# GuildOfWeavers/distaff

Measured on AMD Instinct MI355X. Metric: trace_cells_per_sec, higher is better.
Workload: dtype u128 (prime field 2^128-45*2^40+1, 4x u32 limbs)

## Files before the change

### distaff_amd/csrc/air_kernel.h

```cpp
#pragma once
#include "ctx.h"
#include <type_traits>

#ifndef AIR_THREADS
#define AIR_THREADS 128
#endif
#ifdef AIR_CONVOY
#define AIR_SYNC() __builtin_amdgcn_s_barrier()
#else
#define AIR_SYNC()
#endif
#ifndef AIR_WAVES_PER_SIMD
#define AIR_WAVES_PER_SIMD 2
#endif
constexpr int air_waves_per_simd(int sd, int slcap, int sect) {
    (void)sd; (void)slcap; (void)sect;
#ifdef AIR_WAVES_FORCE
    return AIR_WAVES_FORCE;
#else
    return AIR_WAVES_PER_SIMD;
#endif
}

struct AirConsts { fe sponge_mds[16], sponge_inv_mds[16], hasher_mds[36], hasher_inv_mds[36]; };

struct AirArgs {
    const fe* lde;
    fe* out;
    const fe* coef;
    const fe* tc;
    const fe* periodic;
    const AirConsts* consts;
    fe* partial;
    fe* ev[10];
    const fe* tw_lo; const fe* tw_hi; uint32_t lo_bits;
    unsigned long long* bad_step;
    size_t n, col_stride;
    uint32_t log_n, log_N, log_b, W, ctx_depth, loop_depth, stack_depth;
    uint32_t cl, ll, sl;
    uint32_t coset_step;
    uint32_t q0;
    uint32_t num_inputs, num_outputs;
    fe inputs[8], outputs[8], program_hash[2], op_count;
};



__device__ __forceinline__ fe dpow(const AirArgs& a, uint64_t e) {
    uint32_t l = (uint32_t)e & ((1u << a.lo_bits) - 1u), h = (uint32_t)(e >> a.lo_bits);
    fe v = a.tw_lo[l];
    return h ? fe_mul(v, a.tw_hi[h]) : v;
}

__device__ __forceinline__ fe bnot(const fe& v) { return fe_sub(fe_one(), v); }
__device__ __forceinline__ fe is_bin(const fe& v) { return fe_sub(fe_sqr(v), v); }

template <int Wd>
__device__ __forceinline__ void matmul(fe* s, const fe* m) {
    fe r[Wd];
#pragma unroll
    for (int i = 0; i < Wd; i++) {
        fe_acc A; fe_acc_zero(A);
#pragma unroll
        for (int j = 0; j < Wd; j++) fe_acc_mac(A, m[i * Wd + j], s[j]);
        r[i] = fe_acc_reduce(A);
    }
#pragma unroll
    for (int i = 0; i < Wd; i++) s[i] = r[i];
}

template <int I, int N, class F>
__device__ __forceinline__ void static_for_air(F&& f) {
    if constexpr (I < N) { f(std::integral_constant<int, I>{}); static_for_air<I + 1, N>(f); }
}

struct StackRows { fe o[12], nw[8], hd0; int sl; };
#define ST_AUX0 8
#define ST_AUX1 9

template <int OP, int I> constexpr bool st_has() {
    constexpr bool slot = I < 8, aux0 = I == ST_AUX0, aux1 = I == ST_AUX1;
    switch (OP) {
        case 0x00: case 0x01: case 0x05: case 0x06: case 0x07: return slot || aux0;
        case 0x02: case 0x0E: return slot || aux0;
        case 0x03: case 0x04: case 0x08: case 0x09: case 0x0C: case 0x0D: return slot;
        case 0x0A: case 0x0B: return slot || aux0 || aux1;
        case 0x10: return I >= 1 && slot;
        case 0x11: return I >= 2 && slot;
        case 0x12: case 0x13: case 0x14: case 0x15: return slot;
        case 0x18: return slot && I != 1;
        case 0x19: case 0x1A: case 0x1B: case 0x1C: case 0x1D: return slot;
        default: return false;
    }
}

template <int OP, int I>
__device__ __forceinline__ fe st_term(const StackRows& s) {
    const fe* o = s.o; const fe* nw = s.nw;
    constexpr int i = I < 8 ? I : 0;
    auto L = [&](int num) {
        if (i + num < 8) return fe_sub(o[i + num < 8 ? i + num : 0], nw[i]);
        return i + num < s.sl ? fe_sub(o[i + num < 12 ? i + num : 0], nw[i]) : nw[i];
    };
    auto R = [&](int num) { return fe_sub(o[i - num < 0 ? 0 : i - num], nw[i]); };
    auto C = [&]() { return fe_sub(o[i], nw[i]); };
    auto sel = [&](const fe& c, const fe& x, const fe& y) { return fe_add(y, fe_mul(c, fe_sub(x, y))); };
    if constexpr (OP == 0x00) { if constexpr (I == ST_AUX0) return bnot(o[0]); else return L(1); }
    else if constexpr (OP == 0x01) { if constexpr (I == ST_AUX0) return fe_sub(o[0], o[1]); else return L(2); }
    else if constexpr (OP == 0x02) {
        const fe diff = fe_sub(o[1], o[2]);
        if constexpr (I == ST_AUX0) return fe_mul(nw[0], diff);
        else if constexpr (I == 0) return fe_sub(nw[0], bnot(fe_mul(diff, o[0])));
        else return L(2);
    }
    else if constexpr (OP == 0x03) return L(1);
    else if constexpr (OP == 0x04) return L(4);
    else if constexpr (OP == 0x05) {
        if constexpr (I == ST_AUX0) return is_bin(o[2]);
        else if constexpr (I == 0) return fe_sub(nw[0], sel(o[2], o[0], o[1]));
        else return L(2);
    }
    else if constexpr (OP == 0x06) {
        if constexpr (I == ST_AUX0) return is_bin(o[4]);
        else if constexpr (I == 0) return fe_sub(nw[0], sel(o[4], o[0], o[2]));
// ... 151 lines not shown
        }
        if constexpr ((GROUPS & (AG_RESCR | AG_KEEP)) != 0) {
            const fe keep = fe_sub(o[I < 8 ? I : 0], nw[I < 8 ? I : 0]);
            if constexpr ((GROUPS & AG_RESCR) != 0) { if constexpr (I < 6) fe_acc_mac(outer, h.rescr, h.resc[I < 6 ? I : 0]); else fe_acc_mac(outer, h.rescr, keep); }
            if constexpr ((GROUPS & AG_KEEP) != 0) fe_acc_mac(outer, h.keep, keep);
        }
    }
}

template <int I, uint32_t GROUPS> constexpr bool st_touches() {
    if (I >= 8) return (GROUPS & AG_LOW0) != 0;
    return (GROUPS & (AG_LOW0 | AG_LOW1 | AG_HIGH)) != 0;
}

template <int I, uint32_t GROUPS, int SDK, bool DEEP>
__device__ __forceinline__ fe st_output(const StackRows& s, const fe* lo2, const fe& lo0h, const fe* mid, const fe* top, const StackHigh& h) {
    fe_acc outer; fe_acc_zero(outer);
    static_for_air<0, 2>([&](auto c_) {
        constexpr int c = decltype(c_)::value;
        if constexpr (((GROUPS >> (4 * c)) & 0xFu) != 0) {
            fe_acc middle; fe_acc_zero(middle);
            static_for_air<0, 4>([&](auto b_) {
                constexpr int b = decltype(b_)::value;
                constexpr int base = 4 * b + 16 * c;
                if constexpr ((GROUPS & AG_LOW(c, b)) != 0) {
                    static constexpr StMerge M = st_merge<base, I, SDK, DEEP>();
                    if constexpr (M.n > 0) {
                        fe_acc inner; fe_acc_zero(inner);
                        static_for_air<0, M.n>([&](auto e_) {
                            constexpr int e = decltype(e_)::value;
                            fe cf = (base == 0 && M.lead[e] == 0) ? lo0h : lo2[M.lead[e]];
                            static_for_air<0, 4>([&](auto a_) {
                                constexpr int a = decltype(a_)::value;
                                if constexpr (a != M.lead[e] && M.sgn[e][a] != 0) {
                                    const fe other = (base == 0 && a == 0) ? lo0h : lo2[a];
                                    cf = M.sgn[e][a] > 0 ? fe_add(cf, other) : fe_sub(cf, other);
                                }
                            });
                            constexpr int ii = I < 8 ? I : 0;
                            fe term;
                            if constexpr (M.kind[e] == 1) term = fe_sub(s.o[M.j[e]], s.nw[ii]);
                            else if constexpr (M.kind[e] == 2) term = fe_sub(s.nw[ii], s.o[M.j[e]]);
                            else if constexpr (M.kind[e] == 3) term = s.nw[ii];
                            else if constexpr (M.kind[e] == 4) term = fe_neg(s.nw[ii]);
                            else term = st_term<base + M.lead[e], I>(s);
                            fe_acc_mac(inner, cf, term);
                        });
                        fe_acc_mac(middle, mid[b], fe_acc_reduce(inner));
                    }
                }
            });
            fe_acc_mac(outer, top[c], fe_acc_reduce(middle));
        }
    });
    if constexpr ((GROUPS & AG_HIGH) != 0) st_high_degree<I, GROUPS>(outer, s, h);
    return fe_acc_reduce(outer);
}

template <uint32_t ACC_MASK>
struct Acc {
    fe_acc res_acc;
    fe_acc adj_acc[6];
    fe res, adj[6];
    bool nonzero;
    const fe* tc; uint32_t nc;
    __device__ __forceinline__ void emit(uint32_t cidx, int slot, const fe& d) {
        nonzero |= !fe_is_zero(d);
        fe_acc_mac(res_acc, d, tc[cidx]);
        if ((ACC_MASK >> slot) & 1u) fe_acc_mac(adj_acc[slot], d, tc[nc + cidx]);
        else adj[slot] = fe_add(adj[slot], fe_mul(d, tc[nc + cidx]));
    }
};

template <int CL, int LL, int SD, int SLCAP, int SECT, uint32_t GROUPS, int FLAGS>
__global__ void __launch_bounds__(AIR_THREADS, air_waves_per_simd(SD, SLCAP, SECT)) air_kernel(AirArgs a) {
    constexpr bool FIRST = (FLAGS & AF_FIRST) != 0, LAST = (FLAGS & AF_LAST) != 0, EV_IN = (FLAGS & AF_EV_IN) != 0, EV_OUT = (FLAGS & AF_EV_OUT) != 0;
    constexpr int SL = SD ? (SD > 8 ? SD : 8) : SLCAP;
    constexpr bool DEEP = SD == 0 && SLCAP == 12;
    const int cl = (int)a.cl, ll = (int)a.ll;
    const int sl = SD ? SL : (int)a.sl;
    const int sd = SD ? SD : (int)a.stack_depth;
    const fe* c_sponge_mds = a.consts->sponge_mds; const fe* c_sponge_inv_mds = a.consts->sponge_inv_mds;
    const fe* c_hasher_mds = a.consts->hasher_mds; const fe* c_hasher_inv_mds = a.consts->hasher_inv_mds;
    const size_t k = (size_t)blockIdx.x * AIR_THREADS + threadIdx.x;
    if (k >= a.n) return;
    const uint32_t ql = blockIdx.y;
    const uint32_t qg = a.q0 + ql;
    const uint32_t jl = ql * a.coset_step;
    const size_t kn = (k + 1 == a.n) ? 0 : k + 1;
    const fe* cur_p = a.lde + (size_t)jl * a.n + k;
    const fe* nxt_p = a.lde + (size_t)jl * a.n + kn;
    const size_t cs = a.col_stride;
#define CUR(c) cur_p[(size_t)(c) * cs]
#define NXT(c) nxt_p[(size_t)(c) * cs]

    const uint64_t nmask = ((uint64_t)1 << a.log_N) - 1;
    const uint64_t gi = ((uint64_t)k << a.log_b) + (uint64_t)qg * a.coset_step;
    const uint32_t step = (uint32_t)(((uint64_t)k << 3) + qg);
    const uint64_t n64 = a.n;

    const fe c_opc = CUR(0), n_opc = NXT(0);
    fe c_sp[4], n_sp[4], cf[3], ld[5], hd[2], n_cf[3];
#pragma unroll
    for (int i = 0; i < 4; i++) { c_sp[i] = CUR(1 + i); n_sp[i] = NXT(1 + i); }
#pragma unroll
    for (int i = 0; i < 3; i++) { cf[i] = CUR(5 + i); n_cf[i] = NXT(5 + i); }
#pragma unroll
    for (int i = 0; i < 5; i++) ld[i] = CUR(8 + i);
#pragma unroll
    for (int i = 0; i < 2; i++) hd[i] = CUR(13 + i);
    fe c_ctx[CL], n_ctx[CL], c_lp[LL], n_lp[LL], o[SL], nw[SL];
    {
        uint32_t col = 15;
#pragma unroll
        for (int i = 0; i < CL; i++) { bool on = (uint32_t)i < a.ctx_depth; c_ctx[i] = on ? CUR(col + i) : fe_zero(); n_ctx[i] = on ? NXT(col + i) : fe_zero(); }
        col += a.ctx_depth;
#pragma unroll
        for (int i = 0; i < LL; i++) { bool on = (uint32_t)i < a.loop_depth; c_lp[i] = on ? CUR(col + i) : fe_zero(); n_lp[i] = on ? NXT(col + i) : fe_zero(); }
        col += a.loop_depth;
#pragma unroll
        for (int i = 0; i < SL; i++) { bool on = i < sd; o[i] = on ? CUR(col + i) : fe_zero(); nw[i] = on ? NXT(col + i) : fe_zero(); }
    }

    if constexpr ((SECT & 1) != 0) {
        const fe xp = dpow(a, (gi * (6 * n64 + 2)) & nmask);
        const fe one = fe_one();
#pragma unroll 1
        for (int pass = 0; pass < 2; pass++) {
            const fe* cc = a.coef + pass * 94;
            fe_acc R, A; fe_acc_zero(R); fe_acc_zero(A);
            auto term = [&](const fe& v, uint32_t idx) { fe_acc_mac(R, v, cc[idx]); fe_acc_mac(A, v, cc[idx + 1]); };
            term(pass ? fe_sub(c_opc, a.op_count) : c_opc, 0);
            if (pass == 0) { for (int i = 0; i < 4; i++) term(c_sp[i], 2 + 2 * i); }
            else { for (int i = 0; i < 2; i++) term(fe_sub(c_sp[i], a.program_hash[i]), 2 + 2 * i); }
            for (int i = 0; i < 3; i++) term(pass ? fe_sub(cf[i], one) : cf[i], 10 + 2 * i);
            for (int i = 0; i < 5; i++) term(pass ? fe_sub(ld[i], one) : ld[i], 16 + 2 * i);
            for (int i = 0; i < 2; i++) term(pass ? fe_sub(hd[i], one) : hd[i], 26 + 2 * i);
            for (int i = 0; i < CL; i++) if (i < cl) term(c_ctx[i], 30 + 2 * i);
            for (int i = 0; i < LL; i++) if (i < ll) term(c_lp[i], 62 + 2 * i);
            const uint32_t nio = pass ? a.num_outputs : a.num_inputs;
#pragma unroll
            for (int i = 0; i < 8; i++) if ((uint32_t)i < nio) term(fe_sub(o[i], pass ? a.outputs[i] : a.inputs[i]), 78 + 2 * i);
            const fe adj = fe_acc_reduce(A);
            fe_acc_mac(R, adj, xp);
            a.out[((size_t)pass * gridDim.y + ql) * a.n + k] = fe_acc_reduce(R);
        }
    }

    AIR_SYNC();
    fe cff[8], hdf[4], begin_flag, noop_flag, n_void, assert_flag;
    fe lo2[4], mid[4], top[2];
    {
        fe n0 = bnot(cf[0]), n1 = bnot(cf[1]), n2 = bnot(cf[2]);
        fe t0 = fe_mul(n0, n1), t1 = fe_mul(cf[0], n1), t2 = fe_mul(n0, cf[1]), t3 = fe_mul(cf[0], cf[1]);
        cff[0] = fe_mul(t0, n2); cff[1] = fe_mul(t1, n2); cff[2] = fe_mul(t2, n2); cff[3] = fe_mul(t3, n2);
        cff[4] = fe_mul(t0, cf[2]); cff[5] = fe_mul(t1, cf[2]); cff[6] = fe_mul(t2, cf[2]); cff[7] = fe_mul(t3, cf[2]);
        n_void = fe_mul(fe_mul(n_cf[0], n_cf[1]), n_cf[2]);
        fe l0 = bnot(ld[0]), l1 = bnot(ld[1]), l2 = bnot(ld[2]), l3 = bnot(ld[3]);
        lo2[0] = fe_mul(l0, l1); lo2[1] = fe_mul(ld[0], l1);
        lo2[2] = fe_mul(l0, cf[1]);
        lo2[3] = fe_mul(ld[0], ld[1]);
        mid[0] = fe_mul(l2, l3); mid[1] = fe_mul(ld[2], l3); mid[2] = fe_mul(l2, ld[3]); mid[3] = fe_mul(ld[2], ld[3]);
        top[0] = bnot(ld[4]); top[1] = ld[4];
        fe h0 = bnot(hd[0]), h1 = bnot(hd[1]);
        hdf[0] = fe_mul(h0, h1); hdf[1] = fe_mul(hd[0], h1); hdf[2] = fe_mul(h0, hd[1]); hdf[3] = fe_mul(hd[0], hd[1]);
    }
    auto LDF = [&](int idx) { return fe_mul(fe_mul(lo2[idx & 3], mid[(idx >> 2) & 3]), top[idx >> 4]); };
// ... 319 lines not shown
#pragma unroll
            for (int i = 0; i < 6; i++) agg(i, f, fe_sub(ns[i], os[i]));
            copy_from(6, f);
        }
        }

        const uint32_t sbase = 20 + cl + ll;
        if constexpr ((SECT & 40) != 0) { acc.emit(sbase, 4, aux0); acc.emit(sbase + 1, 4, aux1); }
#pragma unroll
        for (int i = 0; i < SLR; i++) if (i < sd) acc.emit(sbase + 2 + i, 4, ev[i]);
    }
    if constexpr (DEEP && (GROUPS & AG_DEEP) != 0) {
        {
            const uint32_t sbase = 20 + cl + ll;
            const fe lo_all = fe_add(fe_add(lo2[0], lo2[1]), fe_add(lo2[2], lo2[3]));
            fe fl1, fl2, fl4, fr1, fr2, fr4, fcp;
            { fe_acc A; fe_acc_zero(A); fe_acc_mac(A, mid[0], lo2[3]); fe_acc_mac(A, mid[2], lo_all); fl1 = fe_add(fe_mul(top[0], fe_acc_reduce(A)), assert_flag); }
            { fe_acc A; fe_acc_zero(A); fe_acc_mac(A, mid[0], fe_add(lo2[1], lo2[2])); fe_acc_mac(A, mid[1], fe_add(lo2[1], lo2[3])); fl2 = fe_mul(top[0], fe_acc_reduce(A)); }
            fl4 = fe_mul(top[0], fe_mul(mid[1], fe_add(lo2[0], lo2[2])));
            fr1 = fe_add(fe_mul(top[1], fe_mul(mid[0], fe_add(lo2[0], lo2[2]))), hdf[0]);
            { fe_acc A; fe_acc_zero(A); fe_acc_mac(A, mid[0], fe_add(lo2[1], lo2[3])); fe_acc_mac(A, mid[1], lo2[1]); fr2 = fe_mul(top[1], fe_acc_reduce(A)); }
            fr4 = fe_mul(top[1], fe_mul(mid[1], lo2[0]));
            {
                fe_acc A; fe_acc_zero(A); fe_acc_mac(A, mid[2], lo_all); fe_acc_mac(A, mid[3], fe_add(lo2[0], lo2[1]));
                fe_acc B; fe_acc_zero(B); fe_acc_mac(B, top[1], fe_acc_reduce(A)); fe_acc_mac(B, top[0], fe_mul(mid[3], fe_add(fe_add(lo2[0], lo2[1]), lo2[2])));
                fcp = fe_add(fe_add(fe_acc_reduce(B), fe_add(hdf[1], hdf[2])), fe_add(begin_flag, noop_flag));
            }
            const uint32_t scol = 15 + a.ctx_depth + a.loop_depth;
#pragma unroll 1
            for (int i = 8; i < sd; i++) {
                const fe ni = NXT(scol + i);
                auto item = [&](int j) { return CUR(scol + j); };
                auto left = [&](int num) { return i + num < sl ? fe_sub(item(i + num), ni) : ni; };
                fe_acc A; fe_acc_zero(A);
                fe_acc_mac(A, fcp, fe_sub(item(i), ni));
                fe_acc_mac(A, fr1, fe_sub(item(i - 1), ni)); fe_acc_mac(A, fr2, fe_sub(item(i - 2), ni)); fe_acc_mac(A, fr4, fe_sub(item(i - 4), ni));
                fe_acc_mac(A, fl1, left(1)); fe_acc_mac(A, fl2, left(2)); fe_acc_mac(A, fl4, left(4));
                acc.emit(sbase + 2 + i, 4, fe_acc_reduce(A));
            }
        }
    }

    if constexpr (SECT == 1) return;
    const bool on_trace = (qg == 0);
    if (on_trace && k + 1 != a.n && acc.nonzero) atomicMin(a.bad_step, (unsigned long long)k);
    acc.res = fe_acc_reduce(acc.res_acc);
    constexpr bool EMITS_STACK = (SECT & 120) != 0 || (GROUPS & AG_DEEP) != 0 || ((GROUPS & AG_STACK_ALL) != 0 && !EV_OUT);
    constexpr uint32_t USED = ((SECT & 2) ? 0x2Fu : 0u) | ((SECT & 4) ? 0x18u : 0u) | ((SECT & 128) ? 0x04u : 0u) | (EMITS_STACK ? 0x10u : 0u);
#pragma unroll
    for (int i = 0; i < 6; i++) if (((ACC_MASK & USED) >> i) & 1u) acc.adj[i] = fe_add(acc.adj[i], fe_acc_reduce(acc.adj_acc[i]));
    if constexpr (!FIRST) {
        acc.res = fe_add(acc.res, a.partial[pidx]);
#pragma unroll
        for (int i = 0; i < 6; i++) if (LAST || ((USED >> i) & 1u)) acc.adj[i] = fe_add(acc.adj[i], a.partial[(size_t)(i + 1) * pstride + pidx]);
    }
    if constexpr (!LAST) {
        a.partial[pidx] = acc.res;
#pragma unroll
        for (int i = 0; i < 6; i++) if (FIRST || ((USED >> i) & 1u)) a.partial[(size_t)(i + 1) * pstride + pidx] = acc.adj[i];
        return;
    }
    fe t;
    if (on_trace && k + 1 != a.n) {
        t = fe_zero();
    } else {
        const uint32_t degs[6] = {2, 3, 4, 6, 7, 8};
        fe_acc T; fe_acc_zero(T);
        fe_acc_add(T, acc.res);
#pragma unroll
        for (int g = 0; g < 6; g++) {
            uint64_t p = 8 * n64 - 1 - (n64 - 1) * degs[g];
            fe_acc_mac(T, acc.adj[g], dpow(a, (gi * p) & nmask));
        }
        t = fe_acc_reduce(T);
    }
    a.out[((size_t)2 * gridDim.y + ql) * a.n + k] = t;
#undef CUR
#undef NXT
}


template <int CL, int LL, int SD, int SLCAP, int SECT, uint32_t GROUPS, int FLAGS>
static void launch_air(dst_ctx* c, const AirArgs& a, uint32_t Q) {
    dim3 g((unsigned)((c->n + AIR_THREADS - 1) / AIR_THREADS), Q);
    static char name[64];
    if (!name[0]) snprintf(name, sizeof(name), "air_kernel<%d,%d,%d,%d,%d,%u,%d>", CL, LL, SD, SLCAP, SECT, (unsigned)GROUPS, FLAGS);
    constexpr int NS = SD == 4 ? 6 : 10;
    const double units = c->W + ((FLAGS & AF_FIRST) ? 0 : 7) + ((FLAGS & AF_LAST) ? 1 : 7) + ((SECT & 1) ? 2 : 0) + ((FLAGS & AF_EV_IN) ? NS : 0) + ((FLAGS & AF_EV_OUT) ? NS : 0);
    { KScope ks_(c, name, 16.0 * c->n * Q * units, true); hipLaunchKernelGGL((air_kernel<CL, LL, SD, SLCAP, SECT, GROUPS, FLAGS>), g, dim3(AIR_THREADS), 0, c->stream, a); }
}
void air_launch_sd4(dst_ctx* c, const AirArgs& a, uint32_t Q);
void air_launch_small(dst_ctx* c, const AirArgs& a, uint32_t Q);
void air_launch_deep(dst_ctx* c, const AirArgs& a, uint32_t Q);
void air_launch_generic(dst_ctx* c, const AirArgs& a, uint32_t Q);
```

### distaff_amd/csrc/ctx.h

```cpp
#pragma once
#include <hip/hip_runtime.h>
#include <stdint.h>
#include <string.h>
#include <memory>
#include <string>
#include <map>
#include <vector>
#include "fe.h"
#include "../../include/distaff_hip.h"

struct __attribute__((aligned(16))) digest { uint32_t w[8]; };
#define AIR_PERIODIC_STRIDE 29

#ifndef NTT_TW4_PAIRS
#define NTT_TW4_PAIRS 0
#endif
#if NTT_TW4_PAIRS
typedef fe_tw tw4_t;
#else
typedef fe tw4_t;
#endif

#define DST_MAX_FRI_LAYERS 24

struct dst_switch_def { const char* name; bool product; const char* values; const char* what; };
static const dst_switch_def DST_SWITCHES[] = {
    {"DISTAFF_SHARD_DEBUG",        true,  "1",               "stderr line per tree exchange on rank 0; communicators record the order of their collectives (dst_comm_trace)"},
    {"DISTAFF_SHARD_TREE_GATHER",  true,  "1",               "sharded Merkle trees: all-gather of all boundary nodes + upper levels repeated on every rank (BASELINE north_star's all-gather-only form) instead of the k-range all-to-all"},
    {"DISTAFF_SHARD_NO_OVERLAP",   true,  "1",               "sharded prover: every collective on the context's main stream (no second stream / events) also on a stream-ordered transport"},
    {"DISTAFF_COMM_TIMEOUT_S",     true,  "seconds",         "communicators: limit of every host wait behind a collective (default 60; <= 0: none); on expiry the rank aborts the communicator and returns DST_ERR_COMM (dst_comm_set_timeout changes it per handle)"},
    {"DISTAFF_LOCAL_TRANSPORT",    true,  "blocking",        "in-process transport (dst_comm_init_local, dst_prove_sharded_local): drain every rank's stream around each collective instead of the stream-ordered form (events between the ranks' streams, nothing waited for)"},
    {"DISTAFF_TMP_REGS",           true,  "4..W",            "registers per transform launch = size of the staging array (default: as many as 12 GiB hold, at most W)"},
    {"DISTAFF_AIR",                false, "small|deep|generic", "force a more general constraint-kernel instance set than the trace shape needs (generic = per-operation formulation)"},
    {"DISTAFF_BOUNDARY",           false, "eval",            "boundary combinations by evaluation on the 8n domain (the reference's route) instead of coefficient form"},
    {"DISTAFF_COMBINE",            false, "steps",           "combine_polys / DEEP composition as the reference's sequence of whole-array steps instead of the fused passes"},
    {"DISTAFF_NTT",                false, "pre|3pass|reg|lds", "force a transform plan family"},
    {"DISTAFF_NTT_SHAPE",          false, "a,b",             "three-pass plans: log2 of the first two pass lengths"},
    {"DISTAFF_NTT_ORDER",          false, "0",               "first pass of an extension in coset-slow block order"},
    {"DISTAFF_NTT_WAVES",          false, "4|8",             "force the 512- or 1024-lane instances of the LDS passes"},
    {"DISTAFF_NTT_FIXED",          false, "0",               "use the any-shape instances where a shape-compiled one exists"},
    {"DISTAFF_NTT_DIF",            false, "0|1|2",           "first pass of an extension: coset DIT (0), pre-scale + DIF (1), DIT with last-stage twiddles from global memory (2)"},
    {"DISTAFF_NTT_DEBUG",          false, "1",               "print the occupancy of every transform launch shape once"},
    {"DISTAFF_LDE_BATCH",          false, "cols,cosets",     "registers x cosets per transform launch"},
    {"DISTAFF_FOLD8_DFT",          false, "0",               "8n-coefficient extensions without the fused fold + 8-point step"},
    {"DISTAFF_TRACE_BUFFER",       false, "1",               "give the trace its own buffer instead of coset 0 of the extension"},
    {"DISTAFF_MERKLE_LEVEL2_LOG",  false, "k",               "build two tree levels per launch from 2^k nodes on (default 2^15)"},
    {"DISTAFF_MERKLE_LEVELS",      false, "1",               "one launch per tree level"},
    {"DISTAFF_SYN_DIV_TABLES",     false, "1",               "synthetic division by power tables + scan instead of the blocked form"},
    {"DISTAFF_FRI_TAIL",           false, "0|k",             "0: no single-launch tail; k: tail from layers of 2^k elements on"},
    {"DISTAFF_FRI_CHAIN",          false, "0",               "FRI commit phase with a root read-back and a host draw per layer"},
    {"DISTAFF_FRI_REPLICATE_LOG",  false, "k",               "sharded prover: replicate FRI layers from 2^k elements on (default 2^17)"},
    {"DISTAFF_SHARD_FORCE_OVERLAP", false, "1",              "sharded prover: the two-stream choreography of a stream-ordered transport over a blocking one"},
    {"DISTAFF_TEST_STALL_COLLECTIVE", false, "k|k@r",        "communicators: fault injection -- before device collective number k (of rank r only) a kernel holds the stream until the communicator is aborted"},
};
enum : size_t {
    HS_WEIGHTS = 0,
    HS_WEIGHTS_BYTES = (4 * 128 + 4) * 16,
    HS_DEEP = 32768,
    HS_DEEP_HALF = 2048,
    HS_FRI_ROOTS = 40960,
    HS_FRI_SLOTS = 45056,
    HS_FRI_SLOT_BYTES = 800,
    HS_AIR_FLAG = 65536 - 64,
    HS_DRAWS = 65536,
    HS_DRAWS_BYTES = (344 + 160) * 16,
    HS_COMPOSE = 65536 + 8192,
    HS_COMPOSE_BYTES = 516 * 16,
    HS_STATUS = 65536 + 8192 + 8320,
    HS_STATUS_SLOTS = 32,
    HS_TREE_READBACK = 65536 + 8192 + 8320 + 2048,
    HS_TAIL_ROOTS = HS_TREE_READBACK + 1024,
    HS_POW = HS_TAIL_ROOTS + 1024,
    HS_TOTAL = 131072
};
static_assert(HS_WEIGHTS + HS_WEIGHTS_BYTES <= HS_DEEP, "boundary weights overlap the DEEP values");
static_assert(HS_DEEP_HALF >= 128 * 16 && HS_DEEP + 2 * HS_DEEP_HALF <= HS_FRI_ROOTS, "DEEP values: W <= 128 registers");
static_assert(HS_FRI_ROOTS + DST_MAX_FRI_LAYERS * 32 <= HS_FRI_SLOTS, "FRI roots overlap the layer slots");
static_assert(8 * 96 + 32 <= HS_FRI_SLOT_BYTES && HS_FRI_SLOTS + DST_MAX_FRI_LAYERS * HS_FRI_SLOT_BYTES <= HS_AIR_FLAG, "FRI layer slots: G <= 8 ranks, DST_MAX_FRI_LAYERS layers");
static_assert(HS_DRAWS + HS_DRAWS_BYTES <= HS_COMPOSE && HS_COMPOSE + HS_COMPOSE_BYTES <= HS_STATUS && HS_STATUS + HS_STATUS_SLOTS * 64 <= HS_TOTAL, "upload regions overlap");
static_assert(HS_STATUS_SLOTS >= 2 + DST_MAX_FRI_LAYERS, "one status slot per tree exchange of a proof");
static_assert(HS_STATUS + HS_STATUS_SLOTS * 64 <= HS_TREE_READBACK && 8 * 96 + 32 <= 1024 && DST_MAX_FRI_LAYERS * 32 <= 1024 && HS_POW + 64 <= HS_TOTAL, "read-back regions overlap");

#ifdef DISTAFF_TEST_HOOKS
#define DST_TEST_HOOKS 1
#else
#define DST_TEST_HOOKS 0
#endif

enum {
    DST_BUF_POLYS = 0,
    DST_BUF_LDE = 1,
    DST_BUF_TRACE_LEAVES = 2,
    DST_BUF_TRACE_NODES = 3,
    DST_BUF_CEVAL_I = 4,
    DST_BUF_CEVAL_F = 5,
    DST_BUF_CEVAL_T = 6,
    DST_BUF_CPOLY = 7,
    DST_BUF_CEVALS = 8,
    DST_BUF_CNODES = 9,
    DST_BUF_COMP_POLY = 10,
    DST_BUF_COMP_EVALS = 11,
    DST_BUF_FRI_EVALS = 12,
    DST_BUF_FRI_NODES = 13,
    DST_BUF_FRI_LEAVES = 14,
};

struct NttPlan {
    uint32_t log_n = 0, log_n1 = 0, log_n2 = 0;
    uint32_t log_n3 = 0;
    uint32_t tile_a = 1, tile_b = 1;
    uint32_t tile_m = 1;
    bool reg_a = false, reg_b = false;
    uint32_t pre_a = 0, pre_b = 0;
};

struct dst_ctx {
// ... 194 lines not shown
```

### distaff_amd/csrc/kernels_air.hip

```cpp
#include "air_kernel.h"
#include "rescue_constants.h"

#if DST_TEST_HOOKS
void air_launch_generic(dst_ctx* c, const AirArgs& a, uint32_t Q) {
    launch_air<16, 8, 0, 32, 2, 0, AF_FIRST>(c, a, Q);
    if (dst_internal_boundary_by_evaluation(c)) launch_air<16, 8, 0, 32, 1, 0, 0>(c, a, Q);
    launch_air<16, 8, 0, 32, 132, 0, 0>(c, a, Q);
    launch_air<16, 8, 0, 32, 8, 0, 0>(c, a, Q);
    launch_air<16, 8, 0, 32, 32, 0, 0>(c, a, Q);
    launch_air<16, 8, 0, 32, 16, 0, 0>(c, a, Q);
    launch_air<16, 8, 0, 32, 64, 0, AF_LAST>(c, a, Q);
}
#endif


int k_constraint_check(dst_ctx* c, int64_t* bad_step) {
    const unsigned long long res = c->air_flag_host;
    if (res != ~0ull) { if (bad_step) *bad_step = (int64_t)res; return DST_ERR_AIR; }
    if (bad_step) *bad_step = -1;
    return DST_OK;
}
int k_eval_constraints(dst_ctx* c, const fe* coeffs_dev, const fe* tc_dev, int64_t* bad_step, bool defer_check) {
    if (!c->air_consts) {
        AirConsts h;
        memcpy(h.sponge_mds, SPONGE_MDS, sizeof(h.sponge_mds)); memcpy(h.sponge_inv_mds, SPONGE_INV_MDS, sizeof(h.sponge_inv_mds));
        memcpy(h.hasher_mds, HASHER_MDS, sizeof(h.hasher_mds)); memcpy(h.hasher_inv_mds, HASHER_INV_MDS, sizeof(h.hasher_inv_mds));
        HIP_TRY(c, hipMalloc(&c->air_consts, sizeof(AirConsts)));
        HIP_TRY(c, hipMemcpy(c->air_consts, &h, sizeof(AirConsts), hipMemcpyHostToDevice));
    }
    AirArgs a{};
    a.lde = c->lde; a.out = c->ceval; a.coef = coeffs_dev; a.tc = tc_dev; a.periodic = c->periodic; a.consts = (const AirConsts*)c->air_consts; a.partial = c->cwork;
    {
        const size_t per = (size_t)(c->Bc / (c->B / 8)) * c->n;
        if (8 * per > c->Bc * c->tmp_regs * c->n) { c->err = "constraint evaluation: staging buffer too small for the stack partial values"; return DST_ERR_STATE; }
        for (int i = 0; i < 8; i++) a.ev[i] = c->tmp + (size_t)i * per;
        a.ev[8] = c->cpoly; a.ev[9] = c->comp_poly;
    }
    a.tw_lo = c->tw_lo; a.tw_hi = c->tw_hi; a.lo_bits = c->tw_lo_bits;
    a.bad_step = (unsigned long long*)c->d_u64;
    a.n = c->n; a.col_stride = c->Bc * c->n;
    a.log_n = c->log_n; a.log_N = c->log_N; a.log_b = c->log_b; a.W = (uint32_t)c->W;
    a.ctx_depth = c->prm.ctx_depth; a.loop_depth = c->prm.loop_depth; a.stack_depth = (uint32_t)c->stack_depth;
    a.coset_step = (uint32_t)(c->B / 8);
    a.q0 = (uint32_t)(c->j0 / (c->B / 8));
    uint32_t Q = (uint32_t)(c->Bc / (c->B / 8));
    a.num_inputs = c->pub.num_inputs; a.num_outputs = c->pub.num_outputs;
    memcpy(a.inputs, c->pub.inputs, sizeof(a.inputs)); memcpy(a.outputs, c->pub.outputs, sizeof(a.outputs));
    memcpy(a.program_hash, c->program_hash, sizeof(a.program_hash));
    a.op_count = fe_from_u64(c->op_count);
    HIP_TRY(c, hipMemsetAsync(c->d_u64, 0xFF, 8, c->stream));
    const uint32_t cd = c->prm.ctx_depth, lp = c->prm.loop_depth, sd = (uint32_t)c->stack_depth;
    a.cl = cd > 1 ? cd : 1; a.ll = lp > 1 ? lp : 1; a.sl = sd > 8 ? sd : 8;
    const char* force = c->sw("DISTAFF_AIR");
    const bool want_generic = force && !strcmp(force, "generic"), want_small = force && !strcmp(force, "small"), want_deep = force && !strcmp(force, "deep");
    const bool general = want_generic || want_deep;
    if (a.cl <= 2 && a.ll <= 1 && sd == 4 && !general && !want_small) air_launch_sd4(c, a, Q);
    else if (a.cl <= 2 && a.ll <= 1 && sd <= 8 && !general) air_launch_small(c, a, Q);
#if DST_TEST_HOOKS
    else if (want_generic) air_launch_generic(c, a, Q);
#endif
    else air_launch_deep(c, a, Q);
    unsigned long long* flag = c->h_stage ? reinterpret_cast<unsigned long long*>(c->h_stage + HS_AIR_FLAG) : &c->air_flag_host;
    HIP_TRY(c, hipMemcpyAsync(flag, c->d_u64, 8, hipMemcpyDeviceToHost, c->stream));
    if (defer_check && c->h_stage) return DST_OK;
    HIP_TRY(c, hipStreamSynchronize(c->stream));
    c->air_flag_host = *flag;
    return k_constraint_check(c, bad_step);
}
```

Before: 605.6 million.

## Check trace-row transition constraints with a dedicated per-row kernel instead of full AIR chain

On evaluation coset 0 (the trace rows), constraints must vanish, so instead of running the full constraint-kernel chain and combining with coefficients, a new two-part check kernel verifies each row's transitions directly and flags a bad step. The output for that coset is zeroed by memset, the remaining cosets run the normal chain shifted by one coset, and the last block of rows (wraparound) on coset 0 still goes through the chain via a new k0 row offset. This removes the expensive random-linear-combination work on one of the cosets in exchange for extra launches and a large new check kernel whose correctness must match the AIR.

After: 602.5 million. About the same (-0.5%).

```diff
diff --git a/distaff_amd/csrc/air_check_kernel.h b/distaff_amd/csrc/air_check_kernel.h
--- /dev/null
+++ b/distaff_amd/csrc/air_check_kernel.h
@@ -0,0 +1,303 @@
+#pragma once
+#include "air_kernel.h"
+
+#define CK_PUSH 32
+#define CK_CMP 33
+#define CK_RESCR 34
+#define CK_KEEP 35
+
+struct StShape { int from, kind, num; };
+__host__ __device__ constexpr StShape st_shape(int op) {
+    switch (op) {
+        case 0x00: case 0x03: return StShape{0, 2, 1};
+        case 0x01: return StShape{0, 2, 2};
+        case 0x02: case 0x05: return StShape{1, 2, 2};
+        case 0x04: return StShape{0, 2, 4};
+        case 0x06: return StShape{2, 2, 4};
+        case 0x07: return StShape{4, 2, 2};
+        case 0x08: case 0x09: case 0x0A: case 0x0B: return StShape{1, 2, 1};
+        case 0x0C: case 0x0D: case 0x0E: return StShape{1, 1, 0};
+        case 0x10: case 0x12: case CK_PUSH: return StShape{1, 3, 1};
+        case 0x11: case 0x13: case 0x15: return StShape{2, 3, 2};
+        case 0x14: return StShape{4, 3, 4};
+        case 0x18: return StShape{2, 1, 0};
+        case 0x19: case 0x1B: case 0x1D: return StShape{4, 1, 0};
+        case 0x1A: case 0x1C: case CK_CMP: return StShape{8, 1, 0};
+        case CK_RESCR: return StShape{6, 1, 0};
+        case CK_KEEP: return StShape{0, 1, 0};
+        default: return StShape{0, 0, 0};
+    }
+}
+
+__host__ __device__ constexpr bool ck_products(int op) {
+    return op == 0x02 || op == 0x05 || op == 0x06 || op == 0x07 || op == 0x09 || op == 0x0A || op == 0x0B || op == 0x0C || op == 0x0E || op == 0x1D || op == CK_CMP;
+}
+
+template <int OP>
+__device__ __forceinline__ void ck_own_terms(fe* v, const StackRows& s) {
+    static_for_air<0, 10>([&](auto i_) {
+        constexpr int I = decltype(i_)::value;
+        if constexpr (st_has<OP, I>() && (I >= 8 || I < st_shape(OP).from)) v[I] = fe_add(v[I], st_term<OP, I>(s));
+    });
+}
+
+template <int PART>
+__global__ void __launch_bounds__(AIR_THREADS) air_trace_check_kernel(AirArgs a) {
+    const size_t k = (size_t)blockIdx.x * AIR_THREADS + threadIdx.x;
+    if (k + 1 >= a.n) return;
+    const fe* cur_p = a.lde + k;
+    const fe* nxt_p = a.lde + k + 1;
+    const size_t cs = a.col_stride;
+#define CUR(c) cur_p[(size_t)(c) * cs]
+#define NXT(c) nxt_p[(size_t)(c) * cs]
+    const int cl = (int)a.cl, ll = (int)a.ll, sl = (int)a.sl, sd = (int)a.stack_depth;
+    const fe* per = a.periodic + (size_t)(((uint32_t)k << 3) & 127u) * AIR_PERIODIC_STRIDE;
+    const fe zero = fe_zero();
+    bool bad = false;
+
+    uint32_t bits = 0;
+#pragma unroll 1
+    for (int i = 0; i < 10; i++) {
+        const fe b = CUR(5 + i);
+        bad |= !fe_is_zero(is_bin(b));
+        bits |= (fe_add(b, zero).v[0] & 1u) << i;
+    }
+    if (bad) { atomicMin(a.bad_step, (unsigned long long)k); return; }
+    const uint32_t cfm = bits & 7u, ldm = (bits >> 3) & 31u, hdm = bits >> 8;
+    const bool ld0 = (ldm & 1u) != 0, ld1 = (ldm & 2u) != 0, cf1 = (cfm & 2u) != 0, hd0 = (hdm & 1u) != 0;
+    enum { HACC = 0, BEGIN = 1, TEND = 2, FEND = 3, LOOP = 4, WRAP = 5, BREAK = 6, VOID = 7 };
+    const uint32_t lo2 = (uint32_t)(!ld0 && !ld1) | (uint32_t)(ld0 && !ld1) << 1 | (uint32_t)(!ld0 && cf1 ) << 2 | (uint32_t)(ld0 && ld1) << 3;
+    const uint32_t lb = (ldm >> 2) & 3u, lc = ldm >> 4;
+    const bool ldf0 = (lo2 & 1u) && lb == 0 && lc == 0, ldf31 = (lo2 & 8u) && lb == 3 && lc == 1;
+    const bool f_push = hdm == 0 && ld0, f_cmp = hdm == 1, f_rescr = hdm == 2, f_begin = ldf0 && hdm == 0, f_noop = ldf31 && hdm == 3;
+
+    const fe c_opc = CUR(0), n_opc = NXT(0);
+    fe c_sp[4], n_sp[4];
+#pragma unroll
+    for (int i = 0; i < 4; i++) { c_sp[i] = CUR(1 + i); n_sp[i] = NXT(1 + i); }
+    const uint32_t lcol = 15 + a.ctx_depth, scol = lcol + a.loop_depth;
+    auto ctx_cur = [&](int i) { return (uint32_t)i < a.ctx_depth ? CUR(15 + i) : fe_zero(); };
+    auto ctx_nxt = [&](int i) { return (uint32_t)i < a.ctx_depth ? NXT(15 + i) : fe_zero(); };
+    auto lp_cur = [&](int i) { return (uint32_t)i < a.loop_depth ? CUR(lcol + i) : fe_zero(); };
+    auto lp_nxt = [&](int i) { return (uint32_t)i < a.loop_depth ? NXT(lcol + i) : fe_zero(); };
+    StackRows s;
+#pragma unroll
+    for (int i = 0; i < 12; i++) s.o[i] = i < sd ? CUR(scol + i) : fe_zero();
+#pragma unroll
+    for (int i = 0; i < 8; i++) s.nw[i] = i < sd ? NXT(scol + i) : fe_zero();
+    s.hd0 = CUR(13); s.sl = sl;
+
+    if constexpr (PART == 0) {
+        const bool ld_all = ldm == 31u, hd_all = hdm == 3u;
+        bad |= !fe_is_zero(fe_sub(cfm == HACC ? fe_add(c_opc, fe_one()) : c_opc, n_opc));
+        bad |= !fe_is_zero(c_opc) && !ld_all && !hd_all;
+        bad |= cfm != 0 && !(ld_all && hd_all);
+        if (cfm == VOID) {
+            fe n_void = fe_one();
+#pragma unroll 1
+            for (int i = 0; i < 3; i++) n_void = fe_mul(n_void, NXT(5 + i));
+            bad |= !fe_is_zero(bnot(n_void));
+        }
+        fe v = zero;
+        if (cfm == BEGIN || cfm == LOOP || cfm == WRAP || cfm == BREAK) v = per[21];
+        if (cfm == TEND || cfm == FEND) v = per[20];
+        if (f_push) v = fe_add(v, per[22]);
+        bad |= !fe_is_zero(v);
+    }
+
+    if constexpr (PART == 0) {
+    if (cfm == HACC) {
+    } else if (cfm == BEGIN || cfm == LOOP || cfm == WRAP) {
+#pragma unroll
+        for (int i = 0; i < 4; i++) bad |= !fe_is_zero(n_sp[i]);
+    } else if (cfm == BREAK || cfm == VOID) {
+#pragma unroll
+        for (int i = 0; i < 4; i++) bad |= !fe_is_zero(fe_sub(c_sp[i], n_sp[i]));
+    } else {
+        bad |= !fe_is_zero(fe_sub(ctx_cur(0), n_sp[0]));
+        { fe m = n_sp[2]; if (cfm == TEND) m = n_sp[1]; bad |= !fe_is_zero(fe_sub(c_sp[0], m)); }
+        bad |= !fe_is_zero(n_sp[3]);
+    }
+    if (cfm == WRAP || cfm == BREAK) bad |= !fe_is_zero(fe_sub(c_sp[0], lp_cur(0)));
+    if (cfm != HACC) {
+        const bool push = cfm == BEGIN || cfm == LOOP, pop = cfm == TEND || cfm == FEND;
+#pragma unroll 1
+        for (int i = 0; i < cl; i++) {
+            const fe ni = ctx_nxt(i);
+            fe v;
+            if (push) v = fe_sub(i == 0 ? c_sp[0] : ctx_cur(i - 1), ni);
+            else if (pop) v = i + 1 < cl ? fe_sub(ctx_cur(i + 1), ni) : ni;
+            else v = fe_sub(ctx_cur(i), ni);
+            bad |= !fe_is_zero(v);
+        }
+#pragma unroll 1
+        for (int i = 0; i < ll; i++) {
+            const fe ni = lp_nxt(i);
+            fe v = zero;
+            if (cfm == LOOP) { if (i >= 1) v = fe_sub(lp_cur(i - 1), ni); }
+            else if (cfm == BREAK) v = i + 1 < ll ? fe_sub(lp_cur(i + 1), ni) : ni;
+            else v = fe_sub(lp_cur(i), ni);
+            bad |= !fe_is_zero(v);
+        }
+    }
+    }
+
+    fe v[10];
+#pragma unroll
+    for (int i = 0; i < 10; i++) v[i] = zero;
+
+    {
+        constexpr int pass = PART;
+        if (pass == 0 ? cfm == HACC : f_rescr) {
+        const int w = pass ? 6 : 4, depth = pass ? sd : 4;
+        const uint32_t col = pass ? scol : 1u;
+        const fe* per_in = per + (pass ? 8 : 0); const fe* per_out = per + (pass ? 14 : 4);
+        const fe* mds = pass ? a.consts->hasher_mds : a.consts->sponge_mds;
+        const fe* inv_mds = pass ? a.consts->hasher_inv_mds : a.consts->sponge_inv_mds;
+        fe cubes[6];
+#pragma unroll
+        for (int j = 0; j < 6; j++) cubes[j] = zero;
+#pragma unroll 1
+        for (int j = 0; j < w; j++) {
+            const fe cb = fe_cube(fe_add(j < depth ? CUR(col + j) : fe_zero(), per_in[j]));
+            static_for_air<0, 6>([&](auto j_) { constexpr int J = decltype(j_)::value; if (j == J) cubes[J] = cb; });
+        }
+#pragma unroll 1
+        for (int i = 0; i < w; i++) {
+            fe_acc A, B; fe_acc_zero(A); fe_acc_zero(B);
+#pragma unroll 1
+            for (int j = 0; j < w; j++) {
+                fe cb = cubes[0];
+                static_for_air<1, 6>([&](auto j_) { constexpr int J = decltype(j_)::value; if (j == J) cb = cubes[J]; });
+                fe_acc_mac(A, mds[i * w + j], cb);
+                fe_acc_mac(B, inv_mds[i * w + j], j < depth ? NXT(col + j) : fe_zero());
+            }
+            fe os = fe_acc_reduce(A);
+            const fe ns = fe_sub(fe_cube(fe_acc_reduce(B)), per_out[i]);
+            if (pass == 0) {
+                if (i == 0) os = fe_add(os, fe_from_u64(ldm | (hdm << 5)));
+                if (i == 1 && f_push) os = fe_add(os, s.nw[0]);
+                bad |= !fe_is_zero(fe_sub(os, ns));
+            } else {
+                const fe d = fe_sub(ns, os);
+                static_for_air<0, 6>([&](auto i_) { constexpr int I = decltype(i_)::value; if (i == I) v[I] = fe_add(v[I], d); });
+            }
+        }
+        }
+    }
+
+    if constexpr (PART == 1) {
+    uint32_t classes = 0;
+#pragma unroll 1
+    for (int t = 0; t < 9; t++) {
+        int op; bool on;
+        if (t < 4) { op = t + 4 * (int)lb + 16 * (int)lc; on = ((lo2 >> t) & 1u) && (op != 0 || hd0); }
+        else if (t == 4) { op = CK_PUSH; on = f_push; }
+        else if (t == 5) { op = CK_CMP; on = f_cmp; }
+        else if (t == 6) { op = CK_RESCR; on = f_rescr; }
+        else { op = CK_KEEP; on = t == 7 ? f_begin : f_noop; }
+        if (!on) continue;
+        static_for_air<0, 32>([&](auto op_) {
+            constexpr int OP = decltype(op_)::value;
+            if constexpr (st_shape(OP).kind != 0 && !ck_products(OP)) { if (op == OP) ck_own_terms<OP>(v, s); }
+        });
+        if (ck_products(op)) {
+            const fe* o = s.o; const fe* nw = s.nw;
+            const fe one = fe_one();
+            const int rounds = op == CK_CMP ? 3 : 1;
+            fe xy = zero;
+#pragma unroll 1
+            for (int r = 0; r < rounds; r++) {
+                fe x0 = zero, y0 = zero, x1 = zero, y1 = zero, x2 = zero, y2 = zero;
+                if (op == 0x02) { const fe diff = fe_sub(o[1], o[2]); x0 = diff; y0 = o[0]; x1 = nw[0]; y1 = diff; }
+                else if (op == 0x05) { x0 = o[2]; y0 = o[2]; x1 = o[2]; y1 = fe_sub(o[0], o[1]); }
+                else if (op == 0x06) { x0 = o[4]; y0 = o[4]; x1 = o[4]; y1 = fe_sub(o[0], o[2]); x2 = o[4]; y2 = fe_sub(o[1], o[3]); }
+                else if (op == 0x07) { x0 = o[4]; y0 = o[4]; x1 = o[4]; y1 = fe_sub(o[2], o[0]); x2 = o[4]; y2 = fe_sub(o[3], o[1]); }
+                else if (op == 0x09) { x0 = o[0]; y0 = o[1]; }
+                else if (op == 0x0A || op == 0x0B) { x0 = o[0]; y0 = o[1]; x1 = o[0]; y1 = o[0]; x2 = o[1]; y2 = o[1]; }
+                else if (op == 0x0C) { x0 = nw[0]; y0 = o[0]; }
+                else if (op == 0x0E) { x0 = o[0]; y0 = o[0]; }
+                else if (op == 0x1D) { x0 = nw[0]; y0 = nw[0]; x1 = nw[0]; y1 = o[2]; }
+                else if (r == 0) { x0 = nw[1]; y0 = nw[1]; x1 = nw[2]; y1 = nw[2]; x2 = nw[1]; y2 = nw[2]; }
+                else if (r == 1) { x0 = fe_sub(nw[1], xy); y0 = nw[3]; x1 = fe_sub(nw[2], xy); y1 = nw[3]; x2 = bnot(o[5]); y2 = bnot(o[4]); }
+                else { x0 = nw[2]; y0 = o[0]; x1 = nw[1]; y1 = o[0]; }
+                const fe p0 = fe_mul(x0, y0), p1 = fe_mul(x1, y1), p2 = fe_mul(x2, y2);
+                if (op == 0x02) { v[0] = fe_add(v[0], fe_sub(nw[0], bnot(p0))); v[ST_AUX0] = fe_add(v[ST_AUX0], p1); }
+                else if (op == 0x05) { v[ST_AUX0] = fe_add(v[ST_AUX0], fe_sub(p0, o[2])); v[0] = fe_add(v[0], fe_sub(nw[0], fe_add(o[1], p1))); }
+                else if (op == 0x06) {
+                    v[ST_AUX0] = fe_add(v[ST_AUX0], fe_sub(p0, o[4]));
+                    v[0] = fe_add(v[0], fe_sub(nw[0], fe_add(o[2], p1))); v[1] = fe_add(v[1], fe_sub(nw[1], fe_add(o[3], p2)));
+                }
+                else if (op == 0x07) {
+                    v[ST_AUX0] = fe_add(v[ST_AUX0], fe_sub(p0, o[4]));
+                    v[0] = fe_add(v[0], fe_sub(nw[0], fe_add(o[0], p1))); v[1] = fe_add(v[1], fe_sub(nw[1], fe_add(o[1], p2)));
+                    v[2] = fe_add(v[2], fe_sub(nw[2], fe_sub(o[2], p1))); v[3] = fe_add(v[3], fe_sub(nw[3], fe_sub(o[3], p2)));
+                }
+                else if (op == 0x09) v[0] = fe_add(v[0], fe_sub(nw[0], p0));
+                else if (op == 0x0A || op == 0x0B) {
+                    v[0] = fe_add(v[0], fe_sub(nw[0], op == 0x0A ? p0 : fe_sub(fe_add(o[0], o[1]), p0)));
+                    v[ST_AUX0] = fe_add(v[ST_AUX0], fe_sub(p1, o[0])); v[ST_AUX1] = fe_add(v[ST_AUX1], fe_sub(p2, o[1]));
+                }
+                else if (op == 0x0C) v[0] = fe_add(v[0], fe_sub(one, p0));
+                else if (op == 0x0E) { v[ST_AUX0] = fe_add(v[ST_AUX0], fe_sub(p0, o[0])); v[0] = fe_add(v[0], fe_sub(nw[0], bnot(o[0]))); }
+                else if (op == 0x1D) {
+                    v[0] = fe_add(v[0], fe_sub(p0, nw[0])); v[1] = fe_add(v[1], nw[1]);
+                    v[2] = fe_add(v[2], fe_sub(nw[2], fe_double(o[2]))); v[3] = fe_add(v[3], fe_sub(nw[3], fe_add(o[3], p1)));
+                }
+                else if (r == 0) { v[0] = fe_add(v[0], fe_sub(p0, nw[1])); v[1] = fe_add(v[1], fe_sub(p1, nw[2])); xy = p2; }
+                else if (r == 1) {
+                    v[2] = fe_add(v[2], fe_sub(nw[4], fe_add(o[4], p0))); v[3] = fe_add(v[3], fe_sub(nw[5], fe_add(o[5], p1)));
+                    v[6] = fe_add(v[6], fe_sub(nw[3], p2));
+                }
+                else {
+                    v[4] = fe_add(v[4], fe_sub(nw[6], fe_add(o[6], p0))); v[5] = fe_add(v[5], fe_sub(nw[7], fe_add(o[7], p1)));
+                    v[7] = fe_add(v[7], fe_sub(fe_double(nw[0]), o[0]));
+                }
+            }
+        }
+        const StShape sh = st_shape(op);
+        if (sh.kind != 0) classes += 1u << (4 * (sh.kind == 1 ? 0 : (sh.kind == 2 ? 1 : 4) + (sh.num == 4 ? 2 : sh.num == 2 ? 1 : 0)));
+        if (sh.kind != 0) {
+#pragma unroll 1
+            for (int i = sh.from; i < 8 && i < sd; i++) {
+                const fe ni = NXT(scol + i);
+                fe term = ni;
+                if (!(sh.kind == 2 && i + sh.num >= sl)) {
+                    const int j = sh.kind == 1 ? i : sh.kind == 2 ? i + sh.num : i - sh.num;
+                    term = fe_sub(j < sd ? CUR(scol + j) : fe_zero(), ni);
+                }
+                static_for_air<0, 8>([&](auto i_) { constexpr int I = decltype(i_)::value; if (i == I) v[I] = fe_add(v[I], term); });
+            }
+        }
+    }
+#pragma unroll
+    for (int i = 0; i < 8; i++) if (i < sd) bad |= !fe_is_zero(v[i]);
+    bad |= !fe_is_zero(v[ST_AUX0]) || !fe_is_zero(v[ST_AUX1]);
+    auto times = [&](uint32_t count, const fe& term, fe& sum) { for (uint32_t r = 0; r < count; r++) sum = fe_add(sum, term); };
+#pragma unroll 1
+    for (int i = 8; i < sd; i++) {
+        const fe ni = NXT(scol + i);
+        auto item = [&](int j) { return CUR(scol + j); };
+        auto left = [&](int num) { return i + num < sl ? fe_sub(item(i + num), ni) : ni; };
+        fe sum = zero;
+        auto count = [&](int cls) { return (classes >> (4 * cls)) & 15u; };
+        if (count(0)) times(count(0), fe_sub(item(i), ni), sum);
+        if (count(1)) times(count(1), left(1), sum);
+        if (count(2)) times(count(2), left(2), sum);
+        if (count(3)) times(count(3), left(4), sum);
+        if (count(4)) times(count(4), fe_sub(item(i - 1), ni), sum);
+        if (count(5)) times(count(5), fe_sub(item(i - 2), ni), sum);
+        if (count(6)) times(count(6), fe_sub(item(i - 4), ni), sum);
+        bad |= !fe_is_zero(sum);
+    }
+    }
+    if (bad) atomicMin(a.bad_step, (unsigned long long)k);
+#undef CUR
+#undef NXT
+}
+
+static void air_launch_trace_check(dst_ctx* c, const AirArgs& a) {
+    dim3 g((unsigned)((c->n + AIR_THREADS - 1) / AIR_THREADS));
+    { KScope ks_(c, "air_trace_check_kernel<0>", 2.0 * c->W * c->n * 16.0, true); hipLaunchKernelGGL(air_trace_check_kernel<0>, g, dim3(AIR_THREADS), 0, c->stream, a); }
+    { KScope ks_(c, "air_trace_check_kernel<1>", 2.0 * c->W * c->n * 16.0, true); hipLaunchKernelGGL(air_trace_check_kernel<1>, g, dim3(AIR_THREADS), 0, c->stream, a); }
+}
diff --git a/distaff_amd/csrc/air_kernel.h b/distaff_amd/csrc/air_kernel.h
--- a/distaff_amd/csrc/air_kernel.h
+++ b/distaff_amd/csrc/air_kernel.h
@@ -40,6 +40,7 @@
     uint32_t cl, ll, sl;
     uint32_t coset_step;
     uint32_t q0;
+    uint32_t k0;
     uint32_t num_inputs, num_outputs;
     fe inputs[8], outputs[8], program_hash[2], op_count;
 };
@@ -357,7 +358,7 @@
     const int sd = SD ? SD : (int)a.stack_depth;
     const fe* c_sponge_mds = a.consts->sponge_mds; const fe* c_sponge_inv_mds = a.consts->sponge_inv_mds;
     const fe* c_hasher_mds = a.consts->hasher_mds; const fe* c_hasher_inv_mds = a.consts->hasher_inv_mds;
-    const size_t k = (size_t)blockIdx.x * AIR_THREADS + threadIdx.x;
+    const size_t k = (size_t)a.k0 + (size_t)blockIdx.x * AIR_THREADS + threadIdx.x;
     if (k >= a.n) return;
     const uint32_t ql = blockIdx.y;
     const uint32_t qg = a.q0 + ql;
@@ -843,12 +844,16 @@
 
 template <int CL, int LL, int SD, int SLCAP, int SECT, uint32_t GROUPS, int FLAGS>
 static void launch_air(dst_ctx* c, const AirArgs& a, uint32_t Q) {
-    dim3 g((unsigned)((c->n + AIR_THREADS - 1) / AIR_THREADS), Q);
-    static char name[64];
-    if (!name[0]) snprintf(name, sizeof(name), "air_kernel<%d,%d,%d,%d,%d,%u,%d>", CL, LL, SD, SLCAP, SECT, (unsigned)GROUPS, FLAGS);
+    const size_t rows = c->n - a.k0;
+    dim3 g((unsigned)((rows + AIR_THREADS - 1) / AIR_THREADS), Q);
+    static char name[64], name_rows[64];
+    if (!name[0]) {
+        snprintf(name, sizeof(name), "air_kernel<%d,%d,%d,%d,%d,%u,%d>", CL, LL, SD, SLCAP, SECT, (unsigned)GROUPS, FLAGS);
+        snprintf(name_rows, sizeof(name_rows), "%s rows", name);
+    }
     constexpr int NS = SD == 4 ? 6 : 10;
     const double units = c->W + ((FLAGS & AF_FIRST) ? 0 : 7) + ((FLAGS & AF_LAST) ? 1 : 7) + ((SECT & 1) ? 2 : 0) + ((FLAGS & AF_EV_IN) ? NS : 0) + ((FLAGS & AF_EV_OUT) ? NS : 0);
-    { KScope ks_(c, name, 16.0 * c->n * Q * units, true); hipLaunchKernelGGL((air_kernel<CL, LL, SD, SLCAP, SECT, GROUPS, FLAGS>), g, dim3(AIR_THREADS), 0, c->stream, a); }
+    { KScope ks_(c, a.k0 == 0 ? name : name_rows, 16.0 * rows * Q * units, true); hipLaunchKernelGGL((air_kernel<CL, LL, SD, SLCAP, SECT, GROUPS, FLAGS>), g, dim3(AIR_THREADS), 0, c->stream, a); }
 }
 void air_launch_sd4(dst_ctx* c, const AirArgs& a, uint32_t Q);
 void air_launch_small(dst_ctx* c, const AirArgs& a, uint32_t Q);
diff --git a/distaff_amd/csrc/ctx.h b/distaff_amd/csrc/ctx.h
--- a/distaff_amd/csrc/ctx.h
+++ b/distaff_amd/csrc/ctx.h
@@ -32,6 +32,7 @@
     {"DISTAFF_LOCAL_TRANSPORT",    true,  "blocking",        "in-process transport (dst_comm_init_local, dst_prove_sharded_local): drain every rank's stream around each collective instead of the stream-ordered form (events between the ranks' streams, nothing waited for)"},
     {"DISTAFF_TMP_REGS",           true,  "4..W",            "registers per transform launch = size of the staging array (default: as many as 12 GiB hold, at most W)"},
     {"DISTAFF_AIR",                false, "small|deep|generic", "force a more general constraint-kernel instance set than the trace shape needs (generic = per-operation formulation)"},
+    {"DISTAFF_AIR_TRACE",          false, "generic",         "transition constraints on the trace rows (evaluation coset 0) by the constraint-kernel chain over all eight cosets instead of the per-row check kernel"},
     {"DISTAFF_BOUNDARY",           false, "eval",            "boundary combinations by evaluation on the 8n domain (the reference's route) instead of coefficient form"},
     {"DISTAFF_COMBINE",            false, "steps",           "combine_polys / DEEP composition as the reference's sequence of whole-array steps instead of the fused passes"},
     {"DISTAFF_NTT",                false, "pre|3pass|reg|lds", "force a transform plan family"},
diff --git a/distaff_amd/csrc/kernels_air.hip b/distaff_amd/csrc/kernels_air.hip
--- a/distaff_amd/csrc/kernels_air.hip
+++ b/distaff_amd/csrc/kernels_air.hip
@@ -1,4 +1,5 @@
 #include "air_kernel.h"
+#include "air_check_kernel.h"
 #include "rescue_constants.h"
 
 #if DST_TEST_HOOKS
@@ -54,12 +55,29 @@
     const char* force = c->sw("DISTAFF_AIR");
     const bool want_generic = force && !strcmp(force, "generic"), want_small = force && !strcmp(force, "small"), want_deep = force && !strcmp(force, "deep");
     const bool general = want_generic || want_deep;
-    if (a.cl <= 2 && a.ll <= 1 && sd == 4 && !general && !want_small) air_launch_sd4(c, a, Q);
-    else if (a.cl <= 2 && a.ll <= 1 && sd <= 8 && !general) air_launch_small(c, a, Q);
+    auto chain = [&](const AirArgs& aa, uint32_t Ql) {
+        if (aa.cl <= 2 && aa.ll <= 1 && sd == 4 && !general && !want_small) air_launch_sd4(c, aa, Ql);
+        else if (aa.cl <= 2 && aa.ll <= 1 && sd <= 8 && !general) air_launch_small(c, aa, Ql);
 #if DST_TEST_HOOKS
-    else if (want_generic) air_launch_generic(c, a, Q);
+        else if (want_generic) air_launch_generic(c, aa, Ql);
 #endif
-    else air_launch_deep(c, a, Q);
+        else air_launch_deep(c, aa, Ql);
+    };
+    const bool trace_check = a.q0 == 0 && !(DST_TEST_HOOKS && (c->sw_is("DISTAFF_AIR_TRACE", "generic") || dst_internal_boundary_by_evaluation(c)));
+    if (!trace_check) chain(a, Q);
+    else {
+        HIP_TRY(c, hipMemsetAsync(a.out + (size_t)2 * Q * c->n, 0, c->n * sizeof(fe), c->stream));
+        air_launch_trace_check(c, a);
+        if (Q > 1) {
+            AirArgs rest = a;
+            rest.lde += (size_t)a.coset_step * c->n; rest.q0 += 1; rest.out += 3 * c->n;
+            chain(rest, Q - 1);
+        }
+        AirArgs last = a;
+        last.out += (size_t)2 * (Q - 1) * c->n;
+        last.k0 = (uint32_t)(c->n > AIR_THREADS ? c->n - AIR_THREADS : 0);
+        chain(last, 1);
+    }
     unsigned long long* flag = c->h_stage ? reinterpret_cast<unsigned long long*>(c->h_stage + HS_AIR_FLAG) : &c->air_flag_host;
     HIP_TRY(c, hipMemcpyAsync(flag, c->d_u64, 8, hipMemcpyDeviceToHost, c->stream));
     if (defer_check && c->h_stage) return DST_OK;
```
